# nihaomiao/WACV23_TSNet

Measured on AMD Instinct MI355X. Metric: retargeted frames/sec at bs=4, 256x256, n_source=3; max-abs delta vs ref, higher is better.
Workload: dtype f32 (convolutions: fp16 x 2 split of the scaled fp32 operands, 3 exact MFMA products, two-level fp32 accumulate; fp32-class accuracy); 1 GPU; TSNet(label_nc=2,n_blocks=0,n_downsampling=3,n_source=3) forward, fp32, B=4 per GPU, 256x256 (BASELINE.json configs[1]); global_batch=4, parallelism=replicas x1 (batch-sharded, weights broadcast once)

## Files before the change

### wacv23_tsnet_amd/csrc/conv_g64_launch.cpp

```cpp
#include <stdexcept>

#include "conv_g64.hpp"
#include "conv_h2s32.hpp"
#include "kernels.hpp"

namespace tsnet {
namespace {

template <int KS, int BM, int NPROD>
void go(const ConvArgs& a, hipStream_t s) {
    launch_tiles(a.in_alpha ? conv_g64_kernel<KS, BM, NPROD, true> : conv_g64_kernel<KS, BM, NPROD, false>, BM * 4, (size_t)g64_lds_bytes(BM, one_product(NPROD) ? 1 : 2, a.Cin), a, s);
}

template <int NPROD>
void go_np(const ConvArgs& a, const ConvPlan& p, hipStream_t s) {
    if (a.taps == 1 && p.rows == 64) return go<1, 64, NPROD>(a, s);
    if (a.taps == 1 && p.rows == 128) return go<1, 128, NPROD>(a, s);
    if (a.taps == 9 && p.rows == 64) return go<3, 64, NPROD>(a, s);
    if (a.taps == 9 && p.rows == 128) return go<3, 128, NPROD>(a, s);
    plan_not_built(p, NPROD);
}

}

void launch_conv_g64(const ConvArgs& a, const ConvPlan& p, int nprod, hipStream_t s) {
    nprod == 3 ? go_np<3>(a, p, s) : (nprod == kNprodF16 ? go_np<kNprodF16>(a, p, s) : go_np<1>(a, p, s));
}

void launch_conv_h2s32(const ConvArgs& a, int nprod, hipStream_t s) {
    if (nprod == 3) launch_tiles(conv_h2s32_kernel<3>, 256, (size_t)h2s32_lds_bytes(2), a, s);
    else if (nprod == kNprodF16) launch_tiles(conv_h2s32_kernel<kNprodF16>, 256, (size_t)h2s32_lds_bytes(1), a, s);
    else launch_tiles(conv_h2s32_kernel<1>, 256, (size_t)h2s32_lds_bytes(1), a, s);
}

}
```

### wacv23_tsnet_amd/csrc/engine.cpp

```cpp
#include <hip/hip_runtime.h>

#include <algorithm>
#include <cmath>
#include <cstdio>
#include <cstdlib>
#include <cstring>
#include <map>
#include <memory>
#include <stdexcept>
#include <string>
#include <vector>

#include "../../include/tsnet_abi.h"
#include "conv_plan.hpp"
#include "kernels.hpp"
#include "lmfit.hpp"
#include "face_adapt.hpp"
#include "flow_warp.hpp"
#include "frames.hpp"
#include "head_conv.hpp"
#include "norm_elementwise.hpp"
#include "pack_weights.hpp"
#include "postproc.hpp"
#include "raster.hpp"
// ... 244 lines not shown
}

void launch_finalize_impl(const double* part, float* alpha, float* beta, int N, int C, int S, int HW, hipStream_t s) {
    if (S > 8) {
        hipLaunchKernelGGL(in_finalize2_kernel, dim3((C + kFin2Ch - 1) / kFin2Ch, N), dim3(256), 0, s, part, alpha, beta, C, S, HW, 1e-5f);
    } else {
        const int NC = N * C;
        hipLaunchKernelGGL(in_finalize_kernel, dim3((NC + 255) / 256), dim3(256), 0, s, part, alpha, beta, NC, C, S, HW, 1e-5f);
    }
    check_launch("in_finalize");
}

void run_add_stats(Ctx& ctx, const float* x, const float* add, int add_nmod, float* y, int N, int HW, int C, double* part, float* alpha, float* beta, int x_sb = 0,
                   const int* slot = nullptr) {
    if (C & 3) throw ArgError("add_stats: C must be a multiple of 4");
    TimeScope ts(ctx, TSNET_T_STATS);
    const int cq = C / 4, cols = cq < 256 ? cq : 256, R = 256 / cols;
    int S = (HW + R * 8 - 1) / (R * 8);
    if (S > 64) S = 64;
    if (S < 1) S = 1;
    const int rps = (HW + S - 1) / S;
    S = (HW + rps - 1) / rps;
    const int nmod = add_nmod > 0 ? add_nmod : 1;
    if (x_sb < 0 || x_sb > nmod || (x_sb && nmod % x_sb)) throw ArgError("add_stats: the source-batch extent must divide add_nmod");
    AddStatsArgs sa{x, add, y, part, HW, C, S, rps, nmod, x_sb ? x_sb : nmod};
    if (slot) hipLaunchKernelGGL(add_stats_slots_kernel, dim3(S, N, (cq + 255) / 256), dim3(256), 0, ctx.stream, AddStatsSlotArgs{sa, slot});
    else hipLaunchKernelGGL(add_stats_partial_kernel, dim3(S, N, (cq + 255) / 256), dim3(256), 0, ctx.stream, sa);
    check_launch("add_stats_partial");
    launch_finalize(part, alpha, beta, N, C, S, HW, ctx.stream);
}

void run_norm_act(Ctx& ctx, const float* x, const float* alpha, const float* beta, int relu, const float* resid,
                  int N, int HW, int C, float* y) {
    if (C & 3) throw ArgError("norm_act: C must be a multiple of 4");
    TimeScope ts(ctx, TSNET_T_ELEMWISE);
    NormActArgs a{x, alpha, beta, resid, y, HW, C, relu, (size_t)N * HW * C / 4};
    if ((double)HW * C / 4 >= 4294967295.0 || N > 65535) throw ArgError("norm_act: tensor too large");
    size_t per_img4 = (size_t)HW * C / 4, gx = (per_img4 + 255) / 256, cap = std::max<size_t>(1, 4096 / (size_t)N);
    if (gx > cap) gx = cap;
    hipLaunchKernelGGL(norm_act_kernel, dim3((unsigned)gx, N), dim3(256), 0, ctx.stream, a);
    check_launch("norm_act");
}

void run_upsample(Ctx& ctx, const float* x, const float* alpha, const float* beta, int relu, int N, int H, int W, int C, float* y, int x_bf16 = 0, int y_bf16 = 0) {
    if (C & 3) throw ArgError("upsample: C must be a multiple of 4");
    TimeScope ts(ctx, TSNET_T_UPSAMPLE);
    UpsampleArgs a{x, alpha, beta, y, N, H, W, C, relu, x_bf16, y_bf16};
    if (2 * H > 65535 || N > 65535) throw ArgError("upsample: tensor too large");
    const size_t row4 = (size_t)2 * W * C / 4;
    hipLaunchKernelGGL(upsample2x_kernel, dim3((unsigned)std::min<size_t>((row4 + 255) / 256, 64), 2 * H, N), dim3(256), 0, ctx.stream, a);
    check_launch("upsample2x");
}

void launch_head(const HeadArgs& ha, int hh, int ww, int B, hipStream_t s, int cus, int force_rows = 0) {
    if (ha.C % (2 * kHead3Ch) != 0) {
        if (force_rows) throw ArgError("head: the narrow head (C not a multiple of 16) has no tile rows to force");
        const int tiles = ((ww + kHeadT - 1) / kHeadT) * ((hh + kHeadT - 1) / kHeadT);
        hipLaunchKernelGGL(head_conv_kernel, dim3(tiles, B), dim3(256), 0, s, ha);
    } else {
        const int tiles_x = (ww + kHead3T - 1) / kHead3T;
        auto go = [&](auto tr) {
            constexpr int TR = decltype(tr)::value;
            const size_t lds = (size_t)(2 * (head3_patch_f4(TR) + kHead3WtsF4) + ha.C / 2) * sizeof(float4);
            ensure_dynamic_lds(reinterpret_cast<const void*>(head_conv3_kernel<TR>), lds);
            hipLaunchKernelGGL(head_conv3_kernel<TR>, dim3(tiles_x * ((hh + TR - 1) / TR), B), dim3(TR * 16), lds, s, ha);
        };
        const int rows = force_rows ? force_rows : head_rows(B, tiles_x, hh, cus);
        if (rows == 32) go(std::integral_constant<int, 32>{});
        else if (rows == 16) go(std::integral_constant<int, 16>{});
        else go(std::integral_constant<int, 8>{});
    }
    check_launch("head_conv");
    ++g_launch_counters[2];
}

void run_l2norm_split(Ctx& ctx, const float* x, unsigned short* q, int N, int P, int C) {
    if (C & 7) throw ArgError("l2norm: C must be a multiple of 8");
    TimeScope ts(ctx, TSNET_T_ELEMWISE);
    const int Ppad = flow_ppad(P);
    hipLaunchKernelGGL(l2norm_split_kernel, dim3((unsigned)(((size_t)N * Ppad + 3) / 4)), dim3(256), 0, ctx.stream, x, q, N, P, Ppad, C, flow_ksteps(C));
    check_launch("l2norm_split");
}

void run_flow(Ctx& ctx, FlowArgs a, int NB, int variant = 0, const int* slot = nullptr) {
    if (a.C & 7) throw ArgError("flow: C must be a multiple of 8");
    if (a.SB == 0) a.SB = a.B;
    if (a.SB < 1 || a.B % a.SB) throw ArgError("flow: the source-batch extent must divide the batch");
    if (variant < 0 || variant > 2) throw ArgError("flow: variant 0, 1 or 2");
    TimeScope ts(ctx, TSNET_T_FLOW);
    const size_t budget = 160 * 1024;
    const int G = (a.part && a.cnt && NB % a.B == 0 && NB / a.B <= 8 && variant != 1) ? flowp_plan(a.B, a.h, a.w, a.C) : 0;
    if (G) {
        a.K = NB / a.B; a.G = G; a.S = flowp_slices(a.h, a.w);
        try {
            launch_flow_p(a, variant, ctx.stream, slot);
        } catch (const std::invalid_argument& e) { throw ArgError(e.what()); }
        check_launch("flow_p");
        return;
    }
    const int NT = flow_lds_bytes(2, a.h, a.w, a.C) <= budget ? 2 : 1;
    const size_t lds = flow_lds_bytes(NT, a.h, a.w, a.C);
    if (lds > budget) throw ArgError("flow: feature width / position count exceed the LDS budget");
    try {
        launch_flow(a, NT, lds, (unsigned)(flow_ppad(a.P) / (32 * NT) * NB), ctx.stream, slot);
    } catch (const std::invalid_argument& e) { throw ArgError(e.what()); }
    check_launch("flow");
}
// ... 77 lines not shown
        u[4 * i + 3] = (float)g2;
    }
    return u;
}

void linspace_pm1(int n, float* out) {
    if (n == 1) { out[0] = -1.f; return; }
    const float start = -1.f, end = 1.f;
    const float step = (end - start) / (float)(n - 1);
    const int half = n / 2;
    for (int i = 0; i < n; ++i) out[i] = i < half ? fmaf(step, (float)i, start) : fmaf(-step, (float)(n - i - 1), end);
}

void coord_table(int H, int W, float* out) {
    for (int i = 0; i < H; ++i) {
        volatile float ys = (float)i / (float)(H - 1);
        volatile float yy = 2.f * ys - 1.f;
        for (int j = 0; j < W; ++j) {
            volatile float xs = (float)j / (float)(W - 1);
            volatile float xx = 2.f * xs - 1.f;
            volatile float x2 = xx * xx;
            volatile float y2 = yy * yy;
            volatile float ss = x2 + y2;
            float* o = out + ((size_t)i * W + j) * 3;
            o[0] = xx; o[1] = yy; o[2] = sqrtf(ss);
        }
    }
}

}

struct tsnet_engine {
    tsnet_cfg cfg{};
    std::string err;
    bool finalized = false;
    int cus = 256;
    int C = 0, h = 0, w = 0, P = 0, K = 0, Bmax = 0;
    int cp_img = 0, cp_lbl = 0;
    int np = 3;
    bool f16 = false;
    bool st16 = false;

    struct Param { std::string name; std::vector<int64_t> shape; std::vector<float> host; bool loaded = false; };
    std::vector<Param> params;
    std::map<std::string, int> pindex;

    std::vector<ConvLayer> img_enc, lbl_enc;
    ConvLayer fuse_c1_src, fuse_c1_tar;
    ConvLayer fuse_c2, fuse_out, dec_map, dec_head;
    std::vector<ConvLayer> dec_res, dec_up;
    std::vector<ConvLayer*> all_layers;
    float* head_w = nullptr;
    const float* head_bias = nullptr;

    float* wpack = nullptr; size_t wpack_floats = 0;
    float* arena = nullptr; size_t arena_floats = 0;
    float* d_coords = nullptr; float* d_gx = nullptr; float* d_gy = nullptr;
    unsigned* amax = nullptr;
    unsigned* amax_src() const { return amax; }
    unsigned* amax_tar() const { return amax + (size_t)K * Bmax; }
    unsigned* amax_sg() const { return amax + (size_t)(K + 1) * Bmax; }
    unsigned* amax_dec() const { return amax + (size_t)(K + 2) * Bmax; }

    float *x_img = nullptr, *x_lbl = nullptr;
    std::vector<float*> raw_img, raw_lbl;
    float *X = nullptr, *Y1 = nullptr, *Y2 = nullptr;
    float *tar_fea = nullptr, *that = nullptr, *shat = nullptr, *flow = nullptr, *pg = nullptr;
    float *F1 = nullptr, *F2 = nullptr, *zbar = nullptr, *sg = nullptr;
    float* F1s = nullptr;
    float* FT = nullptr;
    float *D = nullptr, *DY1 = nullptr, *DY2 = nullptr;
    std::vector<float*> U, R;
    float* ab[4][2] = {{nullptr}};
    float* ab_side[2][2] = {{nullptr}};
    int ab_rr = 0, ab_side_rr = 0;
    double* part = nullptr;
    double* part_side = nullptr;
    int* fin_counter = nullptr;
    int* fin_counter_side = nullptr;
    int* flow_cnt = nullptr;
    float* flow_part = nullptr;
    hipStream_t side_stream = nullptr;
    hipEvent_t ev_fork = nullptr, ev_join = nullptr, ev_fork2 = nullptr, ev_join2 = nullptr;
    hipEvent_t ev_done = nullptr;
    float* train_ws = nullptr;

    int cached_B = 0;
    bool cached_shared = false;
    float* bbox_copy = nullptr;
    float* tbox = nullptr;
    int last_B = 0;
    int last_SB = 0;
    bool last_shared = false;
    bool bank = false;
    std::vector<char> bank_filled;
    int* slot_tab = nullptr;
    bool last_bank = false;
    int cur_B = 0;
    float src_div[TSNET_MAX_SOURCES];

    Timing timing;

    void add_param(const std::string& name, std::vector<int64_t> shape) {
        pindex[name] = (int)params.size();
        Param p; p.name = name; p.shape = std::move(shape);
        params.push_back(std::move(p));
// ... 57 lines not shown
        }
        return out[0].cin_pad;
    };
    cp_img = enc("img_enc", 3 + c.label_nc, c.enc_blocks, img_enc);
    cp_lbl = enc("lbl_enc", c.label_nc, 0, lbl_enc);
    const int fc = 2 * C;
    fuse_c1_src = make_conv("fuse_net.model.0.conv_block.1", fc, fc, 3, 1, 1, 1);
    fuse_c1_src.name += "[src]"; fuse_c1_src.cin_real = C; fuse_c1_src.cin_pad = conv_cin_pad(C); fuse_c1_src.cin_off = 0;
    fuse_c1_src.kpad = conv_kpad(3, fuse_c1_src.cin_pad);
    fuse_c1_tar = fuse_c1_src; fuse_c1_tar.name = "fuse_net.model.0.conv_block.1[tar]"; fuse_c1_tar.cin_off = C; fuse_c1_tar.bparam.clear();
    fuse_c2 = make_conv("fuse_net.model.0.conv_block.5", fc, fc, 3, 1, 1, 1);
    fuse_out = make_conv("fuse_net.conv", fc, fc / 2, 1, 1, 0, 0);
    dec_map = make_conv("dec.map_conv", 2 * C, C, 1, 1, 0, 0);
    int n = 0;
    for (int i = 0; i < c.n_blocks; ++i) {
        dec_res.push_back(make_conv("dec.model" + std::to_string(n) + ".0.conv_block.1", C, C, 3, 1, 1, 1));
        dec_res.push_back(make_conv("dec.model" + std::to_string(n) + ".0.conv_block.5", C, C, 3, 1, 1, 1));
        ++n;
    }
    for (int i = 0; i < c.n_downsampling; ++i) {
        const int ci = c.ngf << (c.n_downsampling - i);
        dec_up.push_back(make_conv("dec.model" + std::to_string(n) + ".2", ci, ci / 2, 3, 1, 1, 1));
        ++n;
    }
    dec_head = make_conv("dec.model" + std::to_string(n) + ".1", c.ngf, 3, 7, 1, 3, 1);
    auto to_w1 = [&](ConvLayer& L, int hh, int ww) {
        if (np == 1 || !w1_eligible(L.ks, L.stride, L.pad, L.cin_pad, hh, ww)) return;
        L.form = 1; L.kpad = conv_kpad_w1(L.cin_pad);
    };
    for (size_t i = 1 + c.n_downsampling; i < img_enc.size(); ++i) to_w1(img_enc[i], h, w);
    to_w1(fuse_c1_src, h, w); to_w1(fuse_c1_tar, h, w); to_w1(fuse_c2, h, w);
    for (auto& L : dec_res) to_w1(L, h, w);
    if (!dec_up.empty()) to_w1(dec_up[0], 2 * h, 2 * w);
    if (dec_up.size() > 1) to_w1(dec_up[1], 4 * h, 4 * w);
    for (auto& L : img_enc) all_layers.push_back(&L);
    for (auto& L : lbl_enc) all_layers.push_back(&L);
    all_layers.push_back(&fuse_c1_src); all_layers.push_back(&fuse_c1_tar);
    all_layers.push_back(&fuse_c2); all_layers.push_back(&fuse_out);
    all_layers.push_back(&dec_map);
    for (auto& L : dec_res) all_layers.push_back(&L);
    for (auto& L : dec_up) all_layers.push_back(&L);
}

void tsnet_engine::alloc_all(hipStream_t s) {
    const int planes = np == 1 ? 1 : 2;
    size_t off = 0;
    for (ConvLayer* L : all_layers) { L->b_off = off; off += (size_t)round_up(L->cout, 4); }
    dec_head.b_off = off; off += 4;
    off = (off + 63) / 64 * 64;
    const size_t head_off = off;
    off += (size_t)49 * cfg.ngf * 4 + 64;
    off = (off + 63) / 64 * 64;
    const size_t tab_off = off;
    off += round_up((int)all_layers.size(), 64);
    off = (off + 63) / 64 * 64;
    const size_t planes_off = off;
    size_t o16 = 0;
    for (ConvLayer* L : all_layers) { L->w_off = o16; o16 += (size_t)planes * L->kpad * L->npad; o16 = (o16 + 127) / 128 * 128; }
    off += (o16 + 1) / 2;
    wpack_floats = off;
    HIP_TRY(hipMalloc((void**)&wpack, wpack_floats * sizeof(float)));
    HIP_TRY(hipMemsetAsync(wpack, 0, wpack_floats * sizeof(float), s));
    size_t max_w = 0;
    for (ConvLayer* L : all_layers) max_w = std::max(max_w, (size_t)L->cout * L->cin_total * L->ks * (L->form == 1 ? 4 : L->ks));
    max_w = std::max(max_w, (size_t)3 * cfg.ngf * 49);
    float* stage = nullptr;
    HIP_TRY(hipMalloc((void**)&stage, max_w * sizeof(float)));
    unsigned short* planes_base = reinterpret_cast<unsigned short*>(wpack + planes_off);
    for (size_t i = 0; i < all_layers.size(); ++i) {
        ConvLayer* L = all_layers[i];
        const Param& pw = params[pindex[L->wparam]];
        std::vector<float> wino;
        if (L->form == 1) wino = winograd_x_filters(pw.host);
        const std::vector<float>& wsrc = L->form == 1 ? wino : pw.host;
        float mx = 0.f;
        for (float v : wsrc) { const float av = std::fabs(v); if (av > mx) mx = av; }
        if (!std::isfinite(mx)) throw WeightError("parameter '" + L->wparam + "' holds a non-finite value");
        const int sw = ((np != 1 || f16) && mx > 0.f) ? h2_scale_log2(mx) : 0;
        const float unscale = std::ldexp(1.0f, -sw);
        HIP_TRY(hipMemcpyAsync(stage, wsrc.data(), wsrc.size() * sizeof(float), hipMemcpyHostToDevice, s));
        HIP_TRY(hipMemcpyAsync(wpack + tab_off + i, &unscale, sizeof(float), hipMemcpyHostToDevice, s));
        pack_layer(stage, *L, planes_base + L->w_off, f16 ? -1 : planes, std::ldexp(1.0f, sw), s);
        if (!L->bparam.empty()) {
            const Param& pb = params[pindex[L->bparam]];
            HIP_TRY(hipMemcpyAsync(wpack + L->b_off, pb.host.data(), pb.host.size() * sizeof(float), hipMemcpyHostToDevice, s));
        }
        HIP_TRY(hipStreamSynchronize(s));
        L->wq = planes_base + L->w_off;
        L->w_unscale = (np == 1 && !f16) ? nullptr : wpack + tab_off + i;
        L->bias = L->bparam.empty() ? nullptr : wpack + L->b_off;
    }
    {
        const Param& pw = params[pindex[dec_head.wparam]];
        const Param& pb = params[pindex[dec_head.bparam]];
        HIP_TRY(hipMemcpyAsync(stage, pw.host.data(), pw.host.size() * sizeof(float), hipMemcpyHostToDevice, s));
        HIP_TRY(hipMemcpyAsync(wpack + dec_head.b_off, pb.host.data(), pb.host.size() * sizeof(float), hipMemcpyHostToDevice, s));
        head_w = wpack + head_off;
        head_bias = wpack + dec_head.b_off;
        hipLaunchKernelGGL(pack_head_weights_kernel, dim3(64), dim3(256), 0, s, stage, head_w, cfg.ngf);
        check_launch("pack_head_weights");
        HIP_TRY(hipStreamSynchronize(s));
    }
    HIP_TRY(hipFree(stage));
    for (auto& p : params) { std::vector<float>().swap(p.host); }

    const int H = cfg.height, W = cfg.width;
    {
        std::vector<float> t((size_t)H * W * 3), gx(w), gy(h);
        coord_table(H, W, t.data());
        linspace_pm1(w, gx.data());
        linspace_pm1(h, gy.data());
        HIP_TRY(hipMalloc((void**)&d_coords, t.size() * sizeof(float)));
        HIP_TRY(hipMalloc((void**)&d_gx, w * sizeof(float)));
        HIP_TRY(hipMalloc((void**)&d_gy, h * sizeof(float)));
        HIP_TRY(hipMemcpy(d_coords, t.data(), t.size() * sizeof(float), hipMemcpyHostToDevice));
        HIP_TRY(hipMemcpy(d_gx, gx.data(), w * sizeof(float), hipMemcpyHostToDevice));
        HIP_TRY(hipMemcpy(d_gy, gy.data(), h * sizeof(float), hipMemcpyHostToDevice));
    }

    const size_t NB = (size_t)K * Bmax, B = Bmax;
    std::vector<std::pair<float**, size_t>> req;
    auto want = [&](float** p, size_t n) { req.emplace_back(p, (n + 63) & ~(size_t)63); };
    want(&x_img, NB * H * W * cp_img);
    want(&x_lbl, B * H * W * cp_lbl);
    raw_img.assign(cfg.n_downsampling + 1, nullptr);
    raw_lbl.assign(cfg.n_downsampling + 1, nullptr);
    for (int l = 0; l <= cfg.n_downsampling; ++l) {
        const size_t e = (size_t)(H >> l) * (W >> l) * (cfg.ngf << l);
        want(&raw_img[l], NB * e);
        want(&raw_lbl[l], B * e);
    }
    const size_t fe = (size_t)P * C;
    want(&X, NB * fe); want(&Y1, NB * fe); want(&Y2, NB * fe);
    want(&tar_fea, B * fe); want(&that, (flow_plane_halves((int)B, P, C) + 1) / 2); want(&shat, (flow_plane_halves((int)NB, P, C) + 1) / 2); want(&flow, NB * P * 2); want(&pg, B * fe);
    want(&F1, NB * fe * 2); want(&F2, NB * fe * 2); want(&F1s, NB * fe * 2); want(&zbar, B * fe * 2); want(&sg, B * fe); want(&FT, B * fe * 2);
    want(&D, B * fe); want(&DY1, B * fe); want(&DY2, B * fe);
    U.assign(cfg.n_downsampling, nullptr); R.assign(cfg.n_downsampling, nullptr);
    for (int i = 0; i < cfg.n_downsampling; ++i) {
        const size_t sp = (size_t)(h << (i + 1)) * (w << (i + 1));
        want(&U[i], B * sp * (C >> i));
        want(&R[i], B * sp * (C >> (i + 1)));
    }
    for (int i = 0; i < 4; ++i) { want(&ab[i][0], NB * 2 * C); want(&ab[i][1], NB * 2 * C); }
    for (int i = 0; i < 2; ++i) { want(&ab_side[i][0], NB * 2 * C); want(&ab_side[i][1], NB * 2 * C); }
    want(&bbox_copy, NB * H * W);
    float* slot_f = nullptr;
    want(&slot_f, NB);
    if (P >= 2048 && P % 64 == 0) want(&flow_part, 2 * flowp_part_words((int)NB, P, flowp_slices(h, w)));
    size_t part_doubles = NB * 64 * 2 * C * 2;
    for (int l = 0; l <= cfg.n_downsampling; ++l) {
        const size_t hw = (size_t)(H >> l) * (W >> l), tpi = (hw + 63) / 64;
        part_doubles = std::max(part_doubles, stat_part_doubles(NB, tpi, (size_t)std::max(cfg.ngf << l, 2 * C)));
    }
// ... 148 lines not shown
    fa.part = reinterpret_cast<unsigned long long*>(flow_part); fa.cnt = flow_cnt;
    fa.B = B; fa.SB = SB; fa.P = P; fa.C = C; fa.h = h; fa.w = w; fa.H = H; fa.W = W; fa.sy = H / h; fa.sx = W / w;
    run_flow(cx, fa, NB, 0, slot);
    if (out_flow)
        HIP_TRY(hipMemcpyAsync(out_flow, flow, (size_t)NB * P * 2 * sizeof(float), hipMemcpyDeviceToDevice, cx.stream));
    run_warp(cx, X, flow, pg, B, K, h, w, C, SB, slot);
    if (fork) HIP_TRY(hipEventRecord(ev_join2, side_stream));

    const float sqP = std::sqrt((float)P);
    {
        auto s1 = next_ab(ctx);
        auto s2 = next_ab(ctx);
        run_add_stats(ctx, F1s, FT, B, F1, NB, P, 2 * C, part, s1.first, s1.second, SB, slot);
        ConvCall b; b.x = F1; b.alpha = s1.first; b.beta = s1.second; b.relu = 1; b.bound = sqP;
        b.N = NB; b.H = h; b.W = w; b.y = F2;
        conv_stats(ctx, fuse_c2, b, NB, P, s2.first, s2.second);
        run_fuse_tail(ctx, FuseTailArgs{X, tar_fea, F2, s2.first, s2.second, zbar, B, K, P, C, SB}, slot);
        ConvCall c; c.x = zbar; c.bound = enc_bound() + sqP; c.N = B; c.H = h; c.W = w; c.y = sg;
        c.amax_out = amax_sg();
        conv(ctx, fuse_out, c);
    }

    if (fork) HIP_TRY(hipStreamWaitEvent(ctx.stream, ev_join2, 0));
    join2.done = true;
    {
        ConvCall a; a.x = pg; a.x2 = sg; a.csplit = C; a.x2_nmod = B; a.N = B; a.H = h; a.W = w; a.y = D;
        a.in_amax = amax_sg(); a.bound_add = enc_bound();
        a.amax_out = amax_dec();
        conv(ctx, dec_map, a);
    }
    for (int i = 0; i < cfg.n_blocks; ++i)
        resblock(ctx, dec_res[2 * i], dec_res[2 * i + 1], D, 0.f, amax_dec(), (float)i * sqP, DY1, DY2, B, h, w);
    const float* cur = D; const float* cal = nullptr; const float* cbe = nullptr;
    int hh = h, ww = w, cc = C;
    for (int i = 0; i < cfg.n_downsampling; ++i) {
        const float in_bound = std::sqrt((float)(hh * ww));
        run_upsample(ctx, cur, cal, cbe, cal ? 1 : 0, B, hh, ww, cc, U[i], st16 && i > 0, st16);
        hh *= 2; ww *= 2;
        cc /= 2;
        auto st = next_ab(ctx);
        ConvCall a; a.x = U[i]; a.bound = in_bound; a.N = B; a.H = hh; a.W = ww; a.y = R[i];
        a.x_bf16 = st16; a.y_bf16 = st16;
        if (!cal) { a.in_amax = amax_dec(); a.bound_add = (float)cfg.n_blocks * sqP; }
        conv_stats(ctx, dec_up[i], a, B, hh * ww, st.first, st.second);
        cur = R[i]; cal = st.first; cbe = st.second;
    }
    {
        TimeScope ts(ctx, TSNET_T_CONV);
        HeadArgs ha{};
        ha.x = cur; ha.alpha = cal; ha.beta = cbe; ha.w = head_w; ha.bias = head_bias; ha.y = out_rgb;
        ha.N = B; ha.H = hh; ha.W = ww; ha.C = cc; ha.x_bf16 = st16 && cfg.n_downsampling > 0;
        ha.composite = cfg.pose_composite; ha.fore_x0 = 64; ha.fore_x1 = 192;
        for (int c = 0; c < 3; ++c) ha.bg[c] = (-cfg.pose_mean[c]) / 255.0f;
        launch_head(ha, hh, ww, B, ctx.stream, ctx.cus);
    }
    last_B = B; last_SB = SB; last_shared = cached_shared; last_bank = slot != nullptr;
    HIP_TRY(hipEventRecord(ev_done, ctx.stream));
}

#define API_BEGIN(h)                        \
    if (!(h)) return TSNET_ERR_ARG;         \
    try {
#define API_END(h)                                                              \
    } catch (const ArgError& e) { (h)->err = e.what(); return TSNET_ERR_ARG; }   \
      catch (const WeightError& e) { (h)->err = e.what(); return TSNET_ERR_WEIGHT; } \
      catch (const std::bad_alloc&) { (h)->err = "out of host memory"; return TSNET_ERR_NOMEM; } \
      catch (const std::exception& e) { (h)->err = e.what(); return TSNET_ERR_HIP; } \
    return TSNET_OK;

extern "C" {

int tsnet_abi_version(void) { return TSNET_ABI_VERSION; }

int tsnet_create(const tsnet_cfg* cfg, tsnet_handle* out) {
    if (!cfg || !out) { g_create_error = "null argument"; return TSNET_ERR_ARG; }
    *out = nullptr;
    auto bad = [&](const char* m) { g_create_error = m; return TSNET_ERR_ARG; };
    if (cfg->n_source < 1 || cfg->n_source > TSNET_MAX_SOURCES) return bad("n_source must be in 1..8");
    if (cfg->label_nc < 1) return bad("label_nc must be >= 1");
    if (cfg->n_downsampling < 1 || cfg->n_downsampling > 5) return bad("n_downsampling must be in 1..5");
    if (cfg->ngf < 8 || (cfg->ngf & (cfg->ngf - 1))) return bad("ngf must be a power of two >= 8");
    if (cfg->n_blocks < 0 || cfg->enc_blocks < 0) return bad("block counts must be >= 0");
    const int ds = 1 << cfg->n_downsampling;
    if (cfg->height < ds * 2 || cfg->width < ds * 2 || cfg->height % ds || cfg->width % ds)
        return bad("height/width must be multiples of 2^n_downsampling (and at least twice that)");
    if (cfg->max_batch < 1) return bad("max_batch must be >= 1");
    if (cfg->pose_composite && (cfg->height != 256 || cfg->width != 256))
        return bad("pose composite is defined for 256x256 frames only (TSNet_pose.py:277-280)");
    if (cfg->operand_mode < 0 || cfg->operand_mode > 3) return bad("operand_mode must be 0 (fp32-class), 1 (bf16 operands), 2 (bf16 operands + bf16 storage) or 3 (fp16 operands)");
    try {
        tsnet_engine* e = new tsnet_engine();
        e->cfg = *cfg;
        e->K = cfg->n_source; e->Bmax = cfg->max_batch;
        for (int s = 0; s < TSNET_MAX_SOURCES; ++s) e->src_div[s] = 255.0f;
        e->C = cfg->ngf << cfg->n_downsampling;
        e->h = cfg->height / ds; e->w = cfg->width / ds; e->P = e->h * e->w;
        e->np = cfg->operand_mode != 0 ? 1 : 3;
        e->st16 = cfg->operand_mode == 2;
        e->f16 = cfg->operand_mode == 3;
        e->build_layers();
        *out = e;
    } catch (const std::exception& ex) { g_create_error = ex.what(); return TSNET_ERR_NOMEM; }
    return TSNET_OK;
}

const char* tsnet_last_error(tsnet_handle h) { return h ? h->err.c_str() : g_create_error.c_str(); }

// ... 405 lines not shown
                    int ksize, int stride, int pad, int pad_mode, const float* in_alpha, const float* in_beta, int in_relu,
                    float bound, int nprod, int kernel, int tile, float* y, void* stream) {
    OP_BEGIN
    if (!x || !w_oihw || !y) throw ArgError("null tensor");
    if (nprod != 1 && nprod != 3 && nprod != 4 && nprod != TSNET_NPROD_F16) throw ArgError("conv2d op: nprod must be 1 (bf16 operands), 16 (fp16 operands: one fp16 plane), 3 or 4 products");
    hipStream_t s = (hipStream_t)stream;
    Ctx ctx(s, current_device_cus());
    ConvRequest req;
    try { req = decode_tile_code(kernel, tile); } catch (const std::invalid_argument& e) { throw ArgError(e.what()); }
    OpLayer op(w_oihw, bias, Cin, Cout, ksize, stride, pad, pad_mode, nprod, s, kernel == 3 ? 1 : 0);
    ConvCall c; c.x = x; c.alpha = in_alpha; c.beta = in_beta; c.relu = in_relu; c.bound = bound; c.N = N; c.H = H; c.W = W; c.y = y; c.nprod = nprod;
    run_conv(ctx, op.L, c, req);
    HIP_TRY(hipStreamSynchronize(s));
    OP_END
}

int tsnet_op_conv2d_cat(const float* x, const float* x2, int N, int H, int W, int C1, int C2, int x2_nmod, const float* w_oihw, const float* bias, int Cout,
                        int ksize, int stride, int pad, int pad_mode, float bound, int nprod, float* y, void* stream) {
    OP_BEGIN
    if (!x || !x2 || !w_oihw || !y) throw ArgError("null tensor");
    hipStream_t s = (hipStream_t)stream;
    Ctx ctx(s, current_device_cus());
    OpLayer op(w_oihw, bias, C1 + C2, Cout, ksize, stride, pad, pad_mode, nprod, s);
    ConvCall c; c.x = x; c.x2 = x2; c.csplit = C1; c.x2_nmod = x2_nmod; c.bound = bound; c.N = N; c.H = H; c.W = W; c.y = y; c.nprod = nprod;
    run_conv(ctx, op.L, c);
    HIP_TRY(hipStreamSynchronize(s));
    OP_END
}

int tsnet_op_head(const float* x, int N, int H, int W, int C, const float* in_alpha, const float* in_beta, const float* w_oihw, const float* bias,
                  int composite, const float* bg, float* y, void* stream) {
    OP_BEGIN
    if (!x || !w_oihw || !bias || !y) throw ArgError("null tensor");
    if (C < 4 || (C & 3)) throw ArgError("head op: C must be a multiple of 4");
    if (in_alpha && !in_beta) throw ArgError("head op: alpha without beta");
    HeadRequest hr;
    try { hr = decode_head_code(composite); } catch (const std::invalid_argument& e) { throw ArgError(e.what()); }
    hipStream_t s = (hipStream_t)stream;
    const size_t wn = (size_t)3 * C * 49;
    DevBufs mem;
    float* wd = mem.alloc<float>(wn * sizeof(float));
    float* tab = mem.alloc<float>(((size_t)49 * C * 4 + 64) * sizeof(float));
    float* bd = mem.alloc<float>(4 * sizeof(float));
    HIP_TRY(hipMemsetAsync(tab, 0, ((size_t)49 * C * 4 + 64) * sizeof(float), s));
    HIP_TRY(hipMemcpy(wd, w_oihw, wn * sizeof(float), hipMemcpyDefault));
    HIP_TRY(hipMemcpy(bd, bias, 3 * sizeof(float), hipMemcpyDefault));
    hipLaunchKernelGGL(pack_head_weights_kernel, dim3(64), dim3(256), 0, s, wd, tab, C);
    check_launch("pack_head_weights");
    HeadArgs ha{};
    ha.x = x; ha.alpha = in_alpha; ha.beta = in_alpha ? in_beta : nullptr; ha.w = tab; ha.bias = bd; ha.y = y;
    ha.N = N; ha.H = H; ha.W = W; ha.C = C;
    ha.composite = hr.composite; ha.fore_x0 = 64; ha.fore_x1 = 192;
    for (int c = 0; c < 3; ++c) ha.bg[c] = bg ? bg[c] : 0.f;
    launch_head(ha, H, W, N, s, current_device_cus(), hr.rows);
    HIP_TRY(hipStreamSynchronize(s));
    OP_END
}

int tsnet_op_instnorm_stats(const float* x, int N, int HW, int C, float* alpha, float* beta, void* stream) {
    OP_BEGIN
    if (!x || !alpha || !beta) throw ArgError("null tensor");
    Ctx ctx((hipStream_t)stream, current_device_cus());
    DevBufs mem;
    double* part = mem.alloc<double>((size_t)N * 64 * C * 2 * sizeof(double));
    run_stats(ctx, x, N, HW, C, part, alpha, beta);
    HIP_TRY(hipStreamSynchronize(ctx.stream));
    OP_END
}

int tsnet_op_norm_act(const float* x, const float* alpha, const float* beta, int relu, const float* resid,
                      int N, int HW, int C, float* y, void* stream) {
    OP_BEGIN
    if (!x || !y) throw ArgError("null tensor");
    Ctx ctx((hipStream_t)stream, current_device_cus());
    run_norm_act(ctx, x, alpha, beta, relu, resid, N, HW, C, y);
    OP_END
}

int tsnet_op_upsample2x(const float* x, const float* alpha, const float* beta, int relu, int N, int H, int W, int C, float* y, void* stream) {
    OP_BEGIN
    if (!x || !y) throw ArgError("null tensor");
    Ctx ctx((hipStream_t)stream, current_device_cus());
    run_upsample(ctx, x, alpha, beta, relu, N, H, W, C, y);
    OP_END
}

static int* op_slot_table(DevBufs& bufs, const char* op, const int* slots, int n, int n_src) {
    if (!slots) throw ArgError(std::string(op) + ": null slot table");
    if (n_src < 1) throw ArgError(std::string(op) + ": the number of source images must be >= 1");
    for (int i = 0; i < n; ++i)
        if (slots[i] < 0 || slots[i] >= n_src) throw ArgError(std::string(op) + ": slot " + std::to_string(slots[i]) + " is outside the " + std::to_string(n_src) + " source images");
    int* d = bufs.alloc<int>((size_t)n * sizeof(int));
    HIP_TRY(hipMemcpy(d, slots, (size_t)n * sizeof(int), hipMemcpyHostToDevice));
    return d;
}

static void op_flow_impl(const float* tar_fea, const float* src_fea, const float* tar_bbox, const float* src_bbox,
                         int B, int K, int h, int w, int C, int H, int W, float* flow, int variant, int repeat, float* ms_out, hipStream_t stream,
                         const int* slots = nullptr, int n_src = 0) {
    if (!tar_fea || !src_fea || !tar_bbox || !src_bbox || !flow) throw ArgError("null tensor");
    if (B < 1 || K < 1 || K > 8) throw ArgError("flow op: 1 <= K <= 8 sources, B >= 1");
    if (H % h || W % w) throw ArgError("flow op: bbox size must be a multiple of the feature size");
    Ctx ctx(stream, current_device_cus());
    const int P = h * w, NB = K * B;
    DevBufs bufs;
    const int* dslot = slots ? op_slot_table(bufs, "flow op", slots, NB, n_src) : nullptr;
    const int NS = slots ? n_src : NB;
// ... 535 lines not shown
```

### wacv23_tsnet_amd/csrc/kernels.hpp

```cpp
#pragma once
#include <hip/hip_runtime.h>

#include "conv_common.hpp"
#include "conv_plan.hpp"
#include "flow_args.hpp"

namespace tsnet {

void launch_conv_h2(const ConvArgs& a, const ConvPlan& p, int nprod, int abl, int opt, hipStream_t s);
void launch_conv_h2s(const ConvArgs& a, int nprod, hipStream_t s);
void launch_conv_h2d(const ConvArgs& a, const ConvPlan& p, int nprod, hipStream_t s);
void launch_conv_w1(const ConvArgs& a, int nprod, int abl, hipStream_t s);
void launch_conv_h2r(const ConvArgs& a, const ConvPlan& p, int nprod, hipStream_t s);
void launch_conv_g64(const ConvArgs& a, const ConvPlan& p, int nprod, hipStream_t s);
void launch_conv_h2s32(const ConvArgs& a, int nprod, hipStream_t s);

void launch_flow_p(const FlowArgs& a, int variant, hipStream_t s, const int* slot = nullptr);
void launch_flow(const FlowArgs& a, int NT, size_t lds, unsigned grid, hipStream_t s, const int* slot = nullptr);

void ensure_dynamic_lds(const void* kernel, size_t bytes);
template <class Kernel>
void launch_tiles(Kernel k, int threads, size_t lds, const ConvArgs& a, hipStream_t s) {
    ensure_dynamic_lds(reinterpret_cast<const void*>(k), lds);
    hipLaunchKernelGGL(k, dim3(a.tiles_m * a.tiles_n), dim3(threads), lds, s, a);
}

}
```

Measured before the change: 815.4 frames/s.

## Run the 7x7 output head conv on MFMA with split-fp16 folded filter planes

Adds a new head kernel that computes the final 7x7 conv (C->3, tanh, composite) with fp16 MFMA. Weights are packed into a Toeplitz-style table over a 2x4 output patch so the 3 outputs fill 24 of 32 MFMA columns, and both operands are hi/lo fp16 split with three products for fp32-class accuracy. The input norm and ReLU are fused into LDS staging, and the channel range is split across two half-blocks whose partial sums are reduced through LDS. It replaces the scalar FMA head kernel whenever C is a multiple of 16 and an input norm is present. In exchange it adds weight-table memory, wasted MFMA columns, and a fixed 8-row tile choice.

```diff
diff --git a/wacv23_tsnet_amd/csrc/conv_g64_launch.cpp b/wacv23_tsnet_amd/csrc/conv_g64_launch.cpp
--- a/wacv23_tsnet_amd/csrc/conv_g64_launch.cpp
+++ b/wacv23_tsnet_amd/csrc/conv_g64_launch.cpp
@@ -2,6 +2,7 @@
 
 #include "conv_g64.hpp"
 #include "conv_h2s32.hpp"
+#include "head_mfma.hpp"
 #include "kernels.hpp"
 
 namespace tsnet {
@@ -33,4 +34,22 @@
     else launch_tiles(conv_h2s32_kernel<1>, 256, (size_t)h2s32_lds_bytes(1), a, s);
 }
 
+template <int TR>
+static void go_head(const HeadMfmaArgs& a, hipStream_t s) {
+    const size_t lds = head_mfma_lds_bytes(TR, a.C);
+    ensure_dynamic_lds(reinterpret_cast<const void*>(head_mfma_kernel<TR>), lds);
+    hipLaunchKernelGGL(head_mfma_kernel<TR>, dim3(((a.W + 31) / 32) * ((a.H + TR - 1) / TR), a.N), dim3(hm_threads(TR)), lds, s, a);
 }
+
+void launch_head_mfma(const HeadMfmaArgs& a, int rows, hipStream_t s) {
+    if (rows == 32) go_head<32>(a, s);
+    else if (rows == 16) go_head<16>(a, s);
+    else if (rows == 8) go_head<8>(a, s);
+    else throw std::logic_error("head_mfma: tile rows must be 8, 16 or 32");
+}
+
+void pack_head_mfma(const float* w_oihw_dev, int C, float scale, unsigned short* planes, hipStream_t s) {
+    hipLaunchKernelGGL(pack_head_mfma_kernel, dim3(64), dim3(256), 0, s, w_oihw_dev, planes, C, scale);
+}
+
+}
diff --git a/wacv23_tsnet_amd/csrc/engine.cpp b/wacv23_tsnet_amd/csrc/engine.cpp
--- a/wacv23_tsnet_amd/csrc/engine.cpp
+++ b/wacv23_tsnet_amd/csrc/engine.cpp
@@ -320,7 +320,23 @@
     check_launch("upsample2x");
 }
 
-void launch_head(const HeadArgs& ha, int hh, int ww, int B, hipStream_t s, int cus, int force_rows = 0) {
+void launch_head(const HeadArgs& ha, int hh, int ww, int B, hipStream_t s, int cus, int force_rows = 0, const unsigned short* wq = nullptr,
+                 const float* wq_unscale = nullptr) {
+    if (ha.C % (2 * kHead3Ch) == 0 && ha.alpha) {
+        if (!wq || !wq_unscale) throw std::logic_error("head: the folded filter planes are missing");
+        if ((double)B * hh * ww * ha.C * 4 >= 2147483648.0 || B > 65535) throw ArgError("head: tensor too large");
+        HeadMfmaArgs m{};
+        m.x = ha.x; m.alpha = ha.alpha; m.beta = ha.beta; m.wq = wq; m.w_unscale = wq_unscale; m.bias = ha.bias; m.y = ha.y;
+        m.N = B; m.H = hh; m.W = ww; m.C = ha.C; m.composite = ha.composite; m.fore_x0 = ha.fore_x0; m.fore_x1 = ha.fore_x1;
+        for (int c = 0; c < 3; ++c) m.bg[c] = ha.bg[c];
+        m.x_bf16 = ha.x_bf16;
+        const int sa = h2_scale_log2(std::sqrt((float)hh * (float)ww));
+        m.in_scale = std::ldexp(1.0f, sa); m.in_unscale = std::ldexp(1.0f, -sa);
+        launch_head_mfma(m, force_rows ? force_rows : 8, s);
+        check_launch("head_mfma");
+        ++g_launch_counters[2];
+        return;
+    }
     if (ha.C % (2 * kHead3Ch) != 0) {
         if (force_rows) throw ArgError("head: the narrow head (C not a multiple of 16) has no tile rows to force");
         const int tiles = ((ww + kHeadT - 1) / kHeadT) * ((hh + kHeadT - 1) / kHeadT);
@@ -504,6 +520,8 @@
     std::vector<ConvLayer*> all_layers;
     float* head_w = nullptr;
     const float* head_bias = nullptr;
+    unsigned short* head_wq = nullptr;
+    const float* head_wq_unscale = nullptr;
 
     float* wpack = nullptr; size_t wpack_floats = 0;
     float* arena = nullptr; size_t arena_floats = 0;
@@ -667,7 +685,10 @@
     off += (size_t)49 * cfg.ngf * 4 + 64;
     off = (off + 63) / 64 * 64;
     const size_t tab_off = off;
-    off += round_up((int)all_layers.size(), 64);
+    off += round_up((int)all_layers.size() + 1, 64);
+    off = (off + 63) / 64 * 64;
+    const size_t head_planes_off = off;
+    if (cfg.ngf % 16 == 0) off += head_mfma_table_halves(cfg.ngf) / 2;
     off = (off + 63) / 64 * 64;
     const size_t planes_off = off;
     size_t o16 = 0;
@@ -714,6 +735,19 @@
         head_bias = wpack + dec_head.b_off;
         hipLaunchKernelGGL(pack_head_weights_kernel, dim3(64), dim3(256), 0, s, stage, head_w, cfg.ngf);
         check_launch("pack_head_weights");
+        if (cfg.ngf % 16 == 0) {
+            float mx = 0.f;
+            for (float v : pw.host) { const float av = std::fabs(v); if (av > mx) mx = av; }
+            if (!std::isfinite(mx)) throw WeightError("parameter '" + dec_head.wparam + "' holds a non-finite value");
+            const int sw = mx > 0.f ? h2_scale_log2(mx) : 0;
+            const float unscale = std::ldexp(1.0f, -sw);
+            const size_t slot = tab_off + all_layers.size();
+            HIP_TRY(hipMemcpyAsync(wpack + slot, &unscale, sizeof(float), hipMemcpyHostToDevice, s));
+            head_wq = reinterpret_cast<unsigned short*>(wpack + head_planes_off);
+            head_wq_unscale = wpack + slot;
+            pack_head_mfma(stage, cfg.ngf, std::ldexp(1.0f, sw), head_wq, s);
+            check_launch("pack_head_mfma");
+        }
         HIP_TRY(hipStreamSynchronize(s));
     }
     HIP_TRY(hipFree(stage));
@@ -968,7 +1002,7 @@
         ha.N = B; ha.H = hh; ha.W = ww; ha.C = cc; ha.x_bf16 = st16 && cfg.n_downsampling > 0;
         ha.composite = cfg.pose_composite; ha.fore_x0 = 64; ha.fore_x1 = 192;
         for (int c = 0; c < 3; ++c) ha.bg[c] = (-cfg.pose_mean[c]) / 255.0f;
-        launch_head(ha, hh, ww, B, ctx.stream, ctx.cus);
+        launch_head(ha, hh, ww, B, ctx.stream, ctx.cus, 0, head_wq, head_wq_unscale);
     }
     last_B = B; last_SB = SB; last_shared = cached_shared; last_bank = slot != nullptr;
     HIP_TRY(hipEventRecord(ev_done, ctx.stream));
@@ -1480,7 +1514,21 @@
     ha.N = N; ha.H = H; ha.W = W; ha.C = C;
     ha.composite = hr.composite; ha.fore_x0 = 64; ha.fore_x1 = 192;
     for (int c = 0; c < 3; ++c) ha.bg[c] = bg ? bg[c] : 0.f;
-    launch_head(ha, H, W, N, s, current_device_cus(), hr.rows);
+    unsigned short* wq = nullptr; float* un = nullptr;
+    if (C % 16 == 0 && in_alpha) {
+        std::vector<float> hw(wn);
+        HIP_TRY(hipMemcpy(hw.data(), w_oihw, wn * sizeof(float), hipMemcpyDefault));
+        float mx = 0.f;
+        for (float v : hw) mx = std::max(mx, std::fabs(v));
+        const int sw = mx > 0.f ? h2_scale_log2(mx) : 0;
+        const float unscale = std::ldexp(1.0f, -sw);
+        wq = mem.alloc<unsigned short>(head_mfma_table_halves(C) * sizeof(unsigned short));
+        un = mem.alloc<float>(sizeof(float));
+        HIP_TRY(hipMemcpy(un, &unscale, sizeof(float), hipMemcpyHostToDevice));
+        pack_head_mfma(wd, C, std::ldexp(1.0f, sw), wq, s);
+        check_launch("pack_head_mfma");
+    }
+    launch_head(ha, H, W, N, s, current_device_cus(), hr.rows, wq, un);
     HIP_TRY(hipStreamSynchronize(s));
     OP_END
 }
diff --git a/wacv23_tsnet_amd/csrc/head_mfma.hpp b/wacv23_tsnet_amd/csrc/head_mfma.hpp
--- /dev/null
+++ b/wacv23_tsnet_amd/csrc/head_mfma.hpp
@@ -0,0 +1,204 @@
+#pragma once
+#include "kernels.hpp"
+
+namespace tsnet {
+
+constexpr int kHmPitch = 44, kHmPhase = 11;
+constexpr int kHmSteps = 40;
+constexpr int hm_plane_bytes(int TR) { return (TR + 6) * kHmPitch * 16; }
+constexpr int hm_threads(int TR) { return TR == 32 ? 256 : 128; }
+constexpr size_t head_mfma_lds_bytes(int TR, int C) { return (size_t)4 * hm_plane_bytes(TR) + (size_t)2 * C * sizeof(float); }
+static_assert(head_mfma_table_halves(8) == (size_t)kHmSteps * 2 * 64 * 8, "one stage of the table");
+
+template <int TR>
+__global__ __launch_bounds__(hm_threads(TR), 1) void head_mfma_kernel(HeadMfmaArgs a) {
+    static_assert(TR == 32 || TR == 16 || TR == 8, "tile rows");
+    constexpr int MT = TR >= 16 ? 2 : 1;
+    constexpr int WH = TR / 8 / MT;
+    constexpr int TH = WH * 64;
+    constexpr int PRW = TR + 6, PC = 38, PP = PRW * PC;
+    constexpr int PLANE = hm_plane_bytes(TR);
+    constexpr int NT = 2 * TH;
+    constexpr int NPE = (PP * 4 + NT - 1) / NT;
+    constexpr int NBATCH = 2, BE = (NPE + NBATCH - 1) / NBATCH;
+
+    HIP_DYNAMIC_SHARED(__attribute__((aligned(16))) unsigned char, smem_raw)
+    const int half = TSNET_UNIFORM((int)(threadIdx.x / TH));
+    const int tid = threadIdx.x - half * TH;
+    const int lane = tid & 63, li = lane & 31, lh = lane >> 5;
+    const int wv = TSNET_UNIFORM(tid >> 6);
+    unsigned char* tile = smem_raw + half * 2 * PLANE;
+    float* abt = reinterpret_cast<float*>(smem_raw + 4 * PLANE);
+    const int tiles_x = (a.W + 31) / 32;
+    const int n = blockIdx.y;
+    const int bx0 = (blockIdx.x % tiles_x) * 32, by0 = (blockIdx.x / tiles_x) * TR;
+
+#pragma clang loop vectorize(disable) interleave(disable) unroll(disable)
+    for (int i = threadIdx.x; i < 2 * a.C; i += 2 * TH)
+        abt[i] = (i < a.C ? a.alpha[(size_t)n * a.C + i] : a.beta[(size_t)n * a.C + i - a.C]) * a.in_scale;
+
+    const unsigned xbytes = (unsigned)((size_t)a.N * a.H * a.W * a.C * (a.x_bf16 ? 2 : 4));
+    const tsnet_brsrc_t rsx = tsnet_make_brsrc(a.x, xbytes);
+    const unsigned wbytes = (unsigned)(head_mfma_table_halves(a.C) * 2);
+    const tsnet_brsrc_t rsw = tsnet_make_brsrc(a.wq, wbytes);
+
+    const int quad = threadIdx.x & 3;
+    unsigned src_off[NPE];
+#pragma unroll
+    for (int e = 0; e < NPE; ++e) {
+        const int i = ((int)threadIdx.x + e * NT) >> 2;
+        const int p = i < PP ? i : PP - 1;
+        const int py = p / PC, px = p - py * PC;
+        int iy = by0 + py - 3, ix = bx0 + px - 3;
+        iy = iy < 0 ? -iy : iy; iy = iy >= a.H ? 2 * (a.H - 1) - iy : iy;
+        ix = ix < 0 ? -ix : ix; ix = ix >= a.W ? 2 * (a.W - 1) - ix : ix;
+        iy = iy < 0 ? 0 : (iy >= a.H ? a.H - 1 : iy);
+        ix = ix < 0 ? 0 : (ix >= a.W ? a.W - 1 : ix);
+        src_off[e] = (unsigned)((((size_t)n * a.H + iy) * a.W + ix) * a.C * 4 + quad * 16);
+    }
+    auto stage = [&](int sp) __attribute__((always_inline)) {
+        int tx = (int)threadIdx.x;
+        TSNET_OPAQUE_V(tx);
+        const F4 al = *reinterpret_cast<const F4*>(abt + sp * 16 + quad * 4), be = *reinterpret_cast<const F4*>(abt + a.C + sp * 16 + quad * 4);
+#pragma unroll
+        for (int b = 0; b < NBATCH; ++b) {
+            F4 sx[BE];
+#pragma unroll
+            for (int e = 0; e < BE; ++e) {
+                if (b * BE + e < NPE) {
+                    if (a.x_bf16) {
+                        const F2 q = TSNET_BUF_LOAD8(rsx, src_off[b * BE + e] >> 1, (unsigned)(sp * 32));
+                        const unsigned w0 = __builtin_bit_cast(unsigned, q.v[0]), w1 = __builtin_bit_cast(unsigned, q.v[1]);
+                        sx[e].v[0] = __builtin_bit_cast(float, w0 << 16); sx[e].v[1] = __builtin_bit_cast(float, w0 & 0xFFFF0000u);
+                        sx[e].v[2] = __builtin_bit_cast(float, w1 << 16); sx[e].v[3] = __builtin_bit_cast(float, w1 & 0xFFFF0000u);
+                    } else {
+                        sx[e] = TSNET_BUF_LOAD16(rsx, src_off[b * BE + e], (unsigned)(sp * 64));
+                    }
+                }
+            }
+#pragma unroll
+            for (int e = 0; e < BE; ++e) {
+                if (b * BE + e < NPE) {
+                    float t[4];
+#pragma unroll
+                    for (int k = 0; k < 4; ++k) t[k] = __builtin_fmaxf(__builtin_fmaf(sx[e].v[k], al.v[k], be.v[k]), 0.f);
+                    unsigned h0, l0, h1, l1;
+                    TSNET_SPLIT_2PAIRS(t[0], t[1], t[2], t[3], h0, l0, h1, l1);
+                    const int i = (tx + (b * BE + e) * NT) >> 2;
+                    if (i < PP) {
+                        const int py = i / PC, px = i - py * PC;
+                        unsigned char* dst = smem_raw + (quad >> 1) * 2 * PLANE + (py * kHmPitch + (px & 3) * kHmPhase + (px >> 2)) * 16 + (quad & 1) * 8;
+                        uint2 hw2, lw2;
+                        hw2.x = h0; hw2.y = h1; lw2.x = l0; lw2.y = l1;
+                        *reinterpret_cast<uint2*>(dst) = hw2;
+                        *reinterpret_cast<uint2*>(dst + PLANE) = lw2;
+                    }
+                }
+            }
+        }
+    };
+
+    const unsigned char* abase = tile + (((wv * MT * 8 + 2 * (li >> 3)) * kHmPitch + lh * kHmPhase + (li & 7)) * 16);
+    const unsigned vB = (unsigned)(lane * 16);
+    F4 af[2][2][MT], bf[4][2];
+    auto load_b = [&](int set, int g) __attribute__((always_inline)) {
+#pragma unroll
+        for (int p = 0; p < 2; ++p) bf[set][p] = TSNET_BUF_LOAD16(rsw, vB, (unsigned)((g * 2 + p) * 1024));
+    };
+    auto load_a = [&](int set, int t) __attribute__((always_inline)) {
+        const int r = t / 5, jp = t - r * 5;
+        const unsigned char* b = abase + (r * kHmPitch + ((2 * jp) & 3) * kHmPhase + (jp >> 1)) * 16;
+#pragma unroll
+        for (int i = 0; i < MT; ++i)
+#pragma unroll
+            for (int p = 0; p < 2; ++p) af[set][p][i] = *reinterpret_cast<const F4*>(b + p * PLANE + i * 8 * kHmPitch * 16);
+    };
+    f32x16 acc[MT], tot[MT];
+#pragma unroll
+    for (int i = 0; i < MT; ++i)
+#pragma unroll
+        for (int r = 0; r < 16; ++r) { acc[i][r] = 0.f; tot[i][r] = 0.f; }
+    auto product = [&](int sa, int sb, int pa, int pb, bool fresh) __attribute__((always_inline)) {
+#pragma unroll
+        for (int i = 0; i < MT; ++i) {
+            f32x16 c = acc[i];
+            if (fresh) {
+#pragma unroll
+                for (int r = 0; r < 16; ++r) c[r] = 0.f;
+            }
+            acc[i] = TSNET_MFMA_F16(af[sa][pa][i], bf[sb][pb], c);
+        }
+    };
+
+    const int nst = a.C / 8;
+    load_b(0, half * kHmSteps); load_b(1, half * kHmSteps + 1); load_b(2, half * kHmSteps + 2);
+    __syncthreads();
+    for (int stg = half; stg < nst; stg += 2) {
+        stage(stg >> 1);
+        __syncthreads();
+        load_a(0, 0);
+#pragma unroll 1
+        for (int rq = 0; rq < 2; ++rq) {
+#pragma unroll
+            for (int u = 0; u < 20; ++u) {
+                const int t = rq * 20 + u;
+                const int tb = t + 3;
+                load_b((u + 3) & 3, stg * kHmSteps + tb + (tb >= kHmSteps ? kHmSteps : 0));
+                const int ta = t + 1;
+                load_a((u + 1) & 1, ta >= kHmSteps ? 0 : ta);
+                product(u & 1, u & 3, 1, 0, u % 5 == 0);
+                product(u & 1, u & 3, 0, 1, false);
+                product(u & 1, u & 3, 0, 0, false);
+                if (u % 5 == 4) {
+#pragma unroll
+                    for (int i = 0; i < MT; ++i) tot[i] += acc[i];
+                }
+            }
+        }
+        __syncthreads();
+    }
+
+    float* xch = reinterpret_cast<float*>(smem_raw);
+    if (half == 1) {
+#pragma unroll
+        for (int i = 0; i < MT; ++i)
+#pragma unroll
+            for (int r = 0; r < 16; ++r) xch[(i * 16 + r) * TH + tid] = tot[i][r];
+    }
+    __syncthreads();
+    if (half == 1) return;
+    const float unscale = a.in_unscale * a.w_unscale[0];
+    const int o = li % 3, dx = (li / 3) & 3, dy = li / 12;
+    const float bias = li < 24 ? a.bias[o] : 0.f;
+    const float bgv = o == 0 ? a.bg[0] : (o == 1 ? a.bg[1] : a.bg[2]);
+    const size_t hw = (size_t)a.H * a.W;
+#pragma unroll
+    for (int i = 0; i < MT; ++i) {
+#pragma unroll
+        for (int r = 0; r < 16; ++r) {
+            const int m = (r & 3) + 8 * (r >> 2) + 4 * lh;
+            const int oy = by0 + (wv * MT + i) * 8 + 2 * (m >> 3) + dy, ox = bx0 + 4 * (m & 7) + dx;
+            float v = tanhf((tot[i][r] + xch[(i * 16 + r) * TH + tid]) * unscale + bias);
+            if (a.composite && (ox < a.fore_x0 || ox >= a.fore_x1)) v = bgv;
+            if (li < 24 && oy < a.H && ox < a.W) a.y[((size_t)n * 3 + o) * hw + (size_t)oy * a.W + ox] = v;
+        }
+    }
+}
+
+__global__ void pack_head_mfma_kernel(const float* __restrict__ w, unsigned short* __restrict__ out, int C, float scale) {
+    const size_t total = head_mfma_table_halves(C);
+    for (size_t i = (size_t)blockIdx.x * blockDim.x + threadIdx.x; i < total; i += (size_t)gridDim.x * blockDim.x) {
+        const int e = (int)(i & 7), lane = (int)((i >> 3) & 63), plane = (int)((i >> 9) & 1);
+        const int g = (int)(i >> 10), stg = g / kHmSteps, t = g - stg * kHmSteps;
+        const int r = t / 5, j = 2 * (t - r * 5) + (lane >> 5), nn = lane & 31, c = stg * 8 + e;
+        unsigned hi = 0, lo = 0;
+        if (nn < 24) {
+            const int o = nn % 3, dx = (nn / 3) & 3, dy = nn / 12;
+            const int ky = r - dy, kx = j - dx;
+            if (ky >= 0 && ky <= 6 && kx >= 0 && kx <= 6) split_h2(w[((size_t)o * C + c) * 49 + ky * 7 + kx] * scale, hi, lo);
+        }
+        out[i] = (unsigned short)(plane ? lo : hi);
+    }
+}
+
+}
diff --git a/wacv23_tsnet_amd/csrc/kernels.hpp b/wacv23_tsnet_amd/csrc/kernels.hpp
--- a/wacv23_tsnet_amd/csrc/kernels.hpp
+++ b/wacv23_tsnet_amd/csrc/kernels.hpp
@@ -15,6 +15,25 @@
 void launch_conv_g64(const ConvArgs& a, const ConvPlan& p, int nprod, hipStream_t s);
 void launch_conv_h2s32(const ConvArgs& a, int nprod, hipStream_t s);
 
+struct HeadMfmaArgs {
+    const float* x;
+    const float* alpha;
+    const float* beta;
+    const unsigned short* wq;
+    const float* w_unscale;
+    const float* bias;
+    float* y;
+    int N, H, W, C;
+    int composite, fore_x0, fore_x1;
+    float bg[3];
+    int x_bf16;
+    float in_scale, in_unscale;
+};
+
+constexpr size_t head_mfma_table_halves(int C) { return (size_t)(C / 8) * 40 * 2 * 64 * 8; }
+void launch_head_mfma(const HeadMfmaArgs& a, int rows, hipStream_t s);
+void pack_head_mfma(const float* w_oihw_dev, int C, float scale, unsigned short* planes, hipStream_t s);
+
 void launch_flow_p(const FlowArgs& a, int variant, hipStream_t s, const int* slot = nullptr);
 void launch_flow(const FlowArgs& a, int NT, size_t lds, unsigned grid, hipStream_t s, const int* slot = nullptr);
 
```

Result: faster. 825.7 frames/s, median of 6 (+1.3%).
